# Multi-resolution-diffusion-recommender/SDRM

Measured on AMD Instinct MI355X. Metric: denoising-steps/sec (train+sample) on ML-1M latents, higher is better.
Workload: dtype f32; 1 GPU; ML-1M/MLP shaped synthetic latents (C3/C4); latent=340, width=340, hidden_layers=1, global_batch=8192, n_sample=5429, step_mix=15 train : 78 sample per job cycle, rng=philox4x32-10 on device, sampler_row_chains=2, parallelism=user-sharded dp1, collectives=none

## Files before the change

### include/sdrm_hip_debug.h

```cpp
#ifndef SDRM_HIP_DEBUG_H
#define SDRM_HIP_DEBUG_H

#include "sdrm_hip.h"

#ifdef __cplusplus
extern "C" {
#endif

int sdrm_debug_device_check(const char* gcn_arch, int compute_units);

int sdrm_debug_input_layer_args(int n_items, int hidden, int64_t n_rows, int64_t first, int b, int contiguous, float p_drop,
                                uint32_t* thr, float* scale);

int sdrm_debug_latent_args(int hidden, int latent, int b, int64_t row0, int contiguous);

int sdrm_debug_decoder_nll_args(int latent, int hidden, int n_items, int b, int64_t row0, int64_t n_rows, int contiguous);

int sdrm_debug_vae_adam_args(const uint64_t* addr, const int64_t* n, const float* l2_coef, int n_tensors, int64_t step, int has_partials,
                             int64_t l2_capacity, int64_t* chunks_out);

int sdrm_debug_holdout_args(int n_items, int64_t n_rows, int64_t nnz, double test_prop, int64_t n_u, int64_t* m_out);

int sdrm_debug_vae_eval_args(int n_items, int hidden, int latent, int64_t n_rows, int batch, int k, int metric);

enum { SDRM_TILE_AUTO = -1, SDRM_TILE_COUNT = 5 };

int sdrm_debug_set_tile(sdrm_engine* e, int cfg);
int sdrm_debug_set_nt32_rows(sdrm_engine* e, int max_rows, int max_rows_train);
int sdrm_debug_set_skinny(sdrm_engine* e, int on);
int sdrm_debug_set_rowchain(sdrm_engine* e, int mode);
int sdrm_debug_set_rows48(sdrm_engine* e, int mode);
int sdrm_debug_set_rows48_split(sdrm_engine* e, int mode);
int sdrm_debug_rows48_split_available(const sdrm_engine* e);
int sdrm_debug_set_rows48_share(sdrm_engine* e, int on);
int sdrm_debug_set_sample_persist(sdrm_engine* e, int mode);
int sdrm_debug_split_skew(sdrm_engine* e, unsigned skew);
int sdrm_debug_set_wgrad_strips(sdrm_engine* e, int on);
int sdrm_debug_set_dgrad_rows(sdrm_engine* e, int mode);
int sdrm_debug_rowchain_available(const sdrm_engine* e);
int sdrm_debug_set_fused_reverse(sdrm_engine* e, int mode);
int sdrm_debug_set_chains(sdrm_engine* e, int chains);
int sdrm_debug_chains(const sdrm_engine* e);

enum { SDRM_PLAN_PER_LAYER = 0,
       SDRM_PLAN_SKINNY = 1,
       SDRM_PLAN_ROW96 = 2,
       SDRM_PLAN_ROW48 = 3 };
enum { SDRM_PLAN_DGRAD_TILES = 0,
       SDRM_PLAN_DGRAD_ROWS_PER_LAYER = 1,
       SDRM_PLAN_DGRAD_CHAIN = 2,
       SDRM_PLAN_DGRAD_SKINNY_OWN = 3 };
enum { SDRM_SAMPLE_PATH_SKINNY = 0,
       SDRM_SAMPLE_PATH_PERSIST = 1,
       SDRM_SAMPLE_PATH_PER_LAYER = 2 };
int sdrm_debug_last_plan(const sdrm_engine* e, int* train_path, int* parts, int* dgrad, int* sample_path);

int sdrm_debug_set_gradient_buckets(sdrm_engine* e, int buckets);

int sdrm_debug_philox_draws(sdrm_engine* e, uint64_t seed, uint32_t purpose, uint32_t step, int64_t row0, int rows, int quads,
                            float* normals, uint8_t* lowbits, void* stream);

void* sdrm_debug_comm_handle(const sdrm_engine* e);

int sdrm_debug_plan_wgrad(int rows, int n_out, int k_in, int* slices, int* rows_per_slice);

int sdrm_debug_gemm(int variant, int cfg, const float* A, const float* B, float* C, int M, int N, int K, void* stream);
int sdrm_debug_gemm_time(int variant, int cfg, int M, int N, int K, int reps, float* us_out, void* stream);

int sdrm_debug_svd_args(int64_t m, int64_t n, int64_t nnz, int k, int n_iter);
int sdrm_debug_csr_transpose_args(int64_t m, int64_t n, int64_t capacity);
int sdrm_debug_set_csrt_mark(sdrm_engine* e, int mode);
int sdrm_debug_svd_stage(sdrm_engine* e, const int64_t* indptr, const int32_t* indices, const float* data, int64_t n_rows, int64_t n_cols,
                         int64_t nnz, const float* q, float* y_prod, float* y_orth, void* stream);

int sdrm_debug_neumf_args(int n_users, int n_items, int factor, int64_t listed_users, int64_t listed_items);

int sdrm_debug_neumf_train_args(int n_users, int n_items, int factor, int64_t n, int batch, int64_t step0, float p_drop);

int sdrm_debug_neumf_draw_args(int64_t n, int64_t n_hold, int64_t capacity, int with_present, int n_users);

int sdrm_debug_mlp_train_args(int n_users, int n_items, int64_t n, int batch, int64_t step0, float p_drop, int with_grads, const uint64_t* addr,
                              int n_addr);

int sdrm_debug_mlp_eval_args(int n_users, int n_items, int64_t nnz, int64_t n_rows, int rows_listed, int64_t row0, int64_t n, int batch, int with_out,
                             int with_sse, const uint64_t* addr, int n_addr);

#ifdef __cplusplus
}
// ... 3 lines not shown
```

### sdrm_amd/_lib.py

```python
from __future__ import annotations

import ctypes as C
import os

from . import _build

_LIB = None

c_void_p, c_int, c_int64, c_uint64, c_float = C.c_void_p, C.c_int, C.c_int64, C.c_uint64, C.c_float


class TrainRandoms(C.Structure):
    _fields_ = [("noise", c_void_p), ("t", c_void_p), ("keep", c_void_p)]


class VaeDecoder(C.Structure):
    _fields_ = [("w1", c_void_p), ("b1", c_void_p), ("w2", c_void_p), ("b2", c_void_p), ("latent", c_int), ("hidden", c_int),
                ("n_items", c_int)]


class VaeAdamTensor(C.Structure):
    _fields_ = [("p", c_void_p), ("g", c_void_p), ("m", c_void_p), ("v", c_void_p), ("n", c_int64), ("l2_coef", c_float)]


# ... 135 lines not shown
    "sdrm_debug_philox_draws": (c_int, [c_void_p, c_uint64, C.c_uint32, C.c_uint32, c_int64, c_int, c_int, c_void_p, c_void_p, c_void_p]),
    "sdrm_debug_device_check": (c_int, [C.c_char_p, c_int]),
    "sdrm_debug_input_layer_args": (c_int, [c_int, c_int, c_int64, c_int64, c_int, c_int, c_float, C.POINTER(C.c_uint32), C.POINTER(c_float)]),
    "sdrm_debug_latent_args": (c_int, [c_int, c_int, c_int, c_int64, c_int]),
    "sdrm_debug_decoder_nll_args": (c_int, [c_int, c_int, c_int, c_int, c_int64, c_int64, c_int]),
    "sdrm_debug_vae_adam_args": (c_int, [C.POINTER(c_uint64), C.POINTER(c_int64), C.POINTER(c_float), c_int, c_int64, c_int, c_int64,
                                         C.POINTER(c_int64)]),
    "sdrm_debug_vae_eval_args": (c_int, [c_int, c_int, c_int, c_int64, c_int, c_int, c_int]),
    "sdrm_debug_svd_args": (c_int, [c_int64, c_int64, c_int64, c_int, c_int]),
    "sdrm_debug_csr_transpose_args": (c_int, [c_int64, c_int64, c_int64]),
    "sdrm_debug_set_csrt_mark": (c_int, [c_void_p, c_int]),
    "sdrm_debug_svd_stage": (c_int, [c_void_p, c_void_p, c_void_p, c_void_p, c_int64, c_int64, c_int64, c_void_p, c_void_p, c_void_p, c_void_p]),
    "sdrm_debug_neumf_args": (c_int, [c_int, c_int, c_int, c_int64, c_int64]),
    "sdrm_debug_neumf_train_args": (c_int, [c_int, c_int, c_int, c_int64, c_int, c_int64, c_float]),
    "sdrm_debug_neumf_draw_args": (c_int, [c_int64, c_int64, c_int64, c_int, c_int]),
    "sdrm_debug_mlp_train_args": (c_int, [c_int, c_int, c_int64, c_int, c_int64, c_float, c_int, C.POINTER(c_uint64), c_int]),
    "sdrm_debug_mlp_eval_args": (c_int, [c_int, c_int, c_int64, c_int64, c_int, c_int64, c_int64, c_int, c_int, c_int, C.POINTER(c_uint64), c_int]),
    "sdrm_debug_holdout_args": (c_int, [c_int, c_int64, c_int64, C.c_double, c_int64, C.POINTER(c_int64)]),
    "sdrm_debug_set_tile": (c_int, [c_void_p, c_int]),
    "sdrm_debug_set_nt32_rows": (c_int, [c_void_p, c_int, c_int]),
    "sdrm_debug_set_chains": (c_int, [c_void_p, c_int]),
    "sdrm_debug_chains": (c_int, [c_void_p]),
    "sdrm_debug_last_plan": (c_int, [c_void_p, C.POINTER(c_int), C.POINTER(c_int), C.POINTER(c_int), C.POINTER(c_int)]),
    "sdrm_debug_set_fused_reverse": (c_int, [c_void_p, c_int]),
    "sdrm_debug_set_skinny": (c_int, [c_void_p, c_int]),
    "sdrm_debug_set_rowchain": (c_int, [c_void_p, c_int]),
    "sdrm_debug_set_rows48": (c_int, [c_void_p, c_int]),
    "sdrm_debug_set_rows48_split": (c_int, [c_void_p, c_int]),
    "sdrm_debug_rows48_split_available": (c_int, [c_void_p]),
    "sdrm_debug_split_skew": (c_int, [c_void_p, C.c_uint32]),
    "sdrm_debug_set_sample_persist": (c_int, [c_void_p, c_int]),
    "sdrm_debug_set_rows48_share": (c_int, [c_void_p, c_int]),
    "sdrm_debug_rowchain_available": (c_int, [c_void_p]),
    "sdrm_debug_set_wgrad_strips": (c_int, [c_void_p, c_int]),
    "sdrm_debug_set_dgrad_rows": (c_int, [c_void_p, c_int]),
    "sdrm_debug_comm_handle": (c_void_p, [c_void_p]),
    "sdrm_debug_plan_wgrad": (c_int, [c_int, c_int, c_int, C.POINTER(c_int), C.POINTER(c_int)]),
    "sdrm_debug_gemm_time": (c_int, [c_int, c_int, c_int, c_int, c_int, c_int, C.POINTER(c_float), c_void_p]),
    "sdrm_debug_gemm": (c_int, [c_int, c_int, c_void_p, c_void_p, c_void_p, c_int, c_int, c_int, c_void_p]),
}

RNG_EXPLICIT, RNG_PHILOX = 0, 1
STATUS = {0: "SDRM_OK", -1: "SDRM_ERR_ARG", -2: "SDRM_ERR_SHAPE", -3: "SDRM_ERR_HIP", -4: "SDRM_ERR_STATE",
          -5: "SDRM_ERR_NOMEM", -6: "SDRM_ERR_RCCL", -7: "SDRM_ERR_DEVICE"}


def lib_path() -> str:
    return _build.LIB_PATH


def load(build_if_missing: bool = True):
    global _LIB
    if _LIB is not None:
        return _LIB
    try:
        import torch
    except ImportError:
        pass
    path = lib_path()
    override = os.environ.get("SDRM_LIB")
    if override:
        lib = C.CDLL(os.path.abspath(override))
        missing = [name for name in SIGNATURES if not hasattr(lib, name)]
        if missing:
            raise RuntimeError(f"SDRM_LIB={override}: not this ABI, missing {', '.join(missing[:6])}{' ...' if len(missing) > 6 else ''}")
        for name, (res, args) in SIGNATURES.items():
# ... 25 lines not shown
```

### sdrm_amd/csrc/rowchain.h

```cpp
#pragma once
#include <hip/hip_runtime.h>
#include <stdint.h>

#include "bufres.h"
#include "elementwise.h"
#include "gemm.h"
#include "philox.h"
#include "skinny.h"

namespace sdrm {


__host__ __device__ constexpr int rc_lda(int NP) {
  int p = 4;
  while (((NP + p) % 64) != 8 && ((NP + p) % 64) != 24 && ((NP + p) % 64) != 40 && ((NP + p) % 64) != 56) p += 4;
  return NP + p;
}

struct RowChainArgs {
  const float* x0; const float* noise; const int64_t* t; const uint8_t* keep;
  const float* sqrt_ab; const float* one_minus_ab;
  const float* tembP;
  int B, L, T, H;
  int mode; uint32_t seed_lo, seed_hi, step; int64_t row0; float nd;
// ... 65 lines not shown
    lds0 = (uint32_t)(((tid >> 3) * LDA + 4 * (tid & 7)) * 4);
    g0 = (uint32_t)(((tid >> 3) * sld + 4 * (tid & 7)) * 4);
    sl = 0u; sg = 0u; jj = 0;
    gwrap = (uint32_t)(RC_USERS * sld * 4 - (CT - 1) * 128);
  }
  template <int CT, int LDA>
  __device__ __forceinline__ void next() {
    const bool wrap = jj == CT - 1;
    jj = wrap ? 0 : jj + 1;
    sl += wrap ? (uint32_t)(RC_USERS * LDA * 4 - (CT - 1) * 128) : 128u;
    sg += wrap ? gwrap : 128u;
  }
};

template <int CT>
__device__ __forceinline__ void rc_acc_begin(f32x4 (&acc)[3][CT]) {
#pragma unroll
  for (int rt = 0; rt < 3; ++rt)
#pragma unroll
    for (int ct = 0; ct < CT; ++ct) asm volatile("" : "+a"(acc[rt][ct]));
  asm volatile("s_nop 7");
}
template <int CT>
__device__ __forceinline__ void rc_acc_settle(f32x4 (&acc)[3][CT]) {
  asm volatile("s_nop 15\n\ts_nop 15" : "+a"(acc[0][0]));
#pragma unroll
  for (int rt = 0; rt < 3; ++rt)
#pragma unroll
    for (int ct = 0; ct < CT; ++ct)
      if (rt + ct > 0) asm volatile("" : "+a"(acc[rt][ct]));
}

enum { RC_PLAIN = 0, RC_NEXT_LIGHT = 1, RC_LIGHT = 2 };
template <int CT, int LDA, int NS, bool STREAM, bool NT, int MODE = RC_PLAIN, int RTS = RC_USERS>
__device__ __forceinline__ void rc_kstep(f32x4 (&acc)[3][CT], const f32x4 (&ac)[3], const f32x4 (&bc)[CT], f32x4 (&an)[3],
                                         f32x4 (&bn)[CT], brsrc wres, uint32_t wnext, uint32_t lane16, uint32_t anext,
                                         const float* __restrict__ Act, brsrc sres, RcStream& sw) {
  constexpr int NE = MODE == RC_LIGHT ? 1 : 4;
  constexpr int NSLOT = 3 * NE * CT;
  constexpr int P_A = MODE == RC_LIGHT ? 0 : CT, P_S = MODE == RC_LIGHT ? 0 : CT + 3, NPIECE = P_S + (STREAM ? 2 * NS : 0);
  constexpr int STRIDE = NPIECE == 0 ? NSLOT : (NSLOT / NPIECE >= RC_PIECE_STRIDE ? RC_PIECE_STRIDE : (NSLOT / NPIECE >= 1 ? NSLOT / NPIECE : 1));
  static_assert(NPIECE <= NSLOT && NS <= 2, "not enough MFMA slots for the pipeline pieces");
  f32x4 sv0 = {0.f, 0.f, 0.f, 0.f}, sv1 = sv0;
  uint32_t so0 = 0, so1 = 0;
#pragma unroll
  for (int e = 0; e < NE; ++e)
#pragma unroll
  for (int ct = 0; ct < CT; ++ct)
#pragma unroll
  for (int rt = 0; rt < 3; ++rt) {
    const int s = (e * CT + ct) * 3 + rt;
    asm volatile("v_mfma_f32_16x16x4_f32 %0, %1, %2, %0" : "+a"(acc[rt][ct]) : "v"(bc[ct][e]), "v"(ac[rt][e]));
    if (s % STRIDE == 0 && s / STRIDE < NPIECE) {
      const int p = s / STRIDE;
      if (p < P_A) {
        if (!(RC_DIAG & 2)) {
          uint32_t so = wnext + (p / 4) * 4096;
          asm volatile("" : "+s"(so));
          bn[p] = bload4(wres, lane16 + (p % 4) * 1024, so);
        }
      } else if (p < P_S) {
        if (!(RC_DIAG & 4)) {
          uint32_t ao = anext;
          asm volatile("" : "+v"(ao));
          if (MODE == RC_NEXT_LIGHT) an[p - P_A][0] = *reinterpret_cast<const float*>(reinterpret_cast<const char*>(Act) + ao + (p - P_A) * RTS * LDA * 4);
          else an[p - P_A] = *reinterpret_cast<const f32x4*>(reinterpret_cast<const char*>(Act) + ao + (p - P_A) * RTS * LDA * 4);
        }
      } else {
        constexpr int NSD = NS > 0 ? NS : 1;
        const int k = p - P_S, ph = k / NSD, q = k % NSD;
        if (!(RC_DIAG & 1)) {
          f32x4& v = q == 0 ? sv0 : sv1;
          uint32_t& so = q == 0 ? so0 : so1;
          if (ph == 0) {
            uint32_t lo = sw.lds0 + sw.sl;
            asm volatile("" : "+v"(lo));
            v = *reinterpret_cast<const f32x4*>(reinterpret_cast<const char*>(Act) + lo);
            so = sw.sg;
            sw.template next<CT, LDA>();
          } else {
            asm volatile("" : "+s"(so));
            bstore4<NT>(sres, sw.g0, so, v);
          }
        }
      }
    }
    __builtin_amdgcn_sched_barrier(0);
  }
}

__device__ __forceinline__ void block_sum4(double (&v)[4], double* sh ) {
#pragma unroll
  for (int j = 0; j < 4; ++j)
#pragma unroll
    for (int off = 32; off > 0; off >>= 1) v[j] += __shfl_down(v[j], off, 64);
  const int lane = threadIdx.x & 63, wave = threadIdx.x >> 6;
  __syncthreads();
  if (lane == 0) {
#pragma unroll
    for (int j = 0; j < 4; ++j) sh[4 * wave + j] = v[j];
  }
  __syncthreads();
#pragma unroll
  for (int j = 0; j < 4; ++j) v[j] = (sh[j] + sh[4 + j]) + (sh[8 + j] + sh[12 + j]);
}

template <int CT, bool LIGHT = false>
__global__ __launch_bounds__(NTHREADS, 1) void k_row_fwd(const RowChainArgs a) {
  typedef RowChainCfg<CT> C;
  constexpr int NP = C::NP, NCT = C::NCT, KS = C::KS, QP = C::QP, LDA = C::LDA, RT = 3;
  static_assert(KS % 2 == 0, "K-steps are taken in pairs");
  __shared__ __attribute__((aligned(16))) float Act[RC_ROWS * LDA];
  __shared__ int trow[RC_USERS];
  __shared__ double red[16];
  const int tid = threadIdx.x, lane = tid & 63;
  const int wave = __builtin_amdgcn_readfirstlane(tid >> 6);
  const int wr = wave >> 1, wc = wave & 1;
  const int li = lane & 15, lq = lane >> 4;
  const int g = blockIdx.x, u0 = RC_USERS * g;
  const size_t grow0 = (size_t)RC_ROWS * g;
#ifdef RC_STAMPS
  unsigned long long st_[16] = {0};
#endif
  RC_STAMP(0);

  if (tid < RC_USERS) {
    const int usr = u0 + tid;
    int t0 = 0;
    if (usr < a.B) {
      t0 = train_timestep(a.mode, a.t, a.row0, usr, a.step, a.seed_lo, a.seed_hi, a.T);
      a.tdev[usr] = t0;
    }
    trow[tid] = t0;
  }
  constexpr int NQ = QP / 8;
  const int su = tid >> 3, sq = tid & 7;
  const int susr = u0 + su;
  float4 xs[NQ];
#pragma unroll
  for (int j = 0; j < NQ; ++j) {
    const int c = 4 * (sq + 8 * j);
    xs[j] = (susr < a.B && c < a.L) ? load4_unpadded(a.x0, susr, c, a.L) : make_float4(0.f, 0.f, 0.f, 0.f);
  }
  __syncthreads();
  {
    const int TPc = a.K0 - a.LPs;
    const int TQ8 = TPc >> 5;
    const bool uin = susr < a.B;
    const float* trow_p = a.tembP + (size_t)(uin ? trow[su] : 0) * TPc + 4 * sq;
    const brsrc ures = make_brsrc(a.U + grow0 * a.K0, (uint32_t)(RC_ROWS * a.K0 * 4));
    const uint32_t uvo = (uint32_t)((su * a.K0 + a.LPs + 4 * sq) * 4);
    for (int jq = 0; jq < TQ8; ++jq) {
      const float4 te = uin ? *reinterpret_cast<const float4*>(trow_p + 32 * jq) : make_float4(0.f, 0.f, 0.f, 0.f);
      const f32x4 oh = {te.x, te.y, te.z, te.w};
#pragma unroll
      for (int pass = 0; pass < 3; ++pass) bstore4<true>(ures, uvo, (uint32_t)((pass * RC_USERS * a.K0 + 32 * jq) * 4), oh);
    }
  }
  {
    const int tt = trow[su];
    const float sa = a.sqrt_ab[tt], om = a.one_minus_ab[tt];
    U4 rw[NQ];
    if (a.mode != 0) {
#pragma unroll
      for (int j = 0; j < NQ; ++j)
        rw[j] = train_quad_draw(a.row0, susr, sq + 8 * j, a.step, a.seed_lo, a.seed_hi);
    }
#pragma unroll
    for (int j = 0; j < NQ; ++j) {
      const int c = 4 * (sq + 8 * j);
      float vP[4] = {0.f, 0.f, 0.f, 0.f}, vS[4] = {0.f, 0.f, 0.f, 0.f}, vQ[4] = {0.f, 0.f, 0.f, 0.f};
      if (susr < a.B && c < a.L) {
        const float x_[4] = {xs[j].x, xs[j].y, xs[j].z, xs[j].w};
        float e[4] = {0.f, 0.f, 0.f, 0.f};
        uint32_t bits[4] = {0u, 0u, 0u, 0u};
        if (a.mode != 0) {
          train_quad_decode(rw[j], a.nd, e, bits);
        }
#pragma unroll
        for (int k = 0; k < 4; ++k) {
          if (c + k < a.L) {
            const size_t idx = (size_t)susr * a.L + c + k;
            const float x = x_[k];
            bool k1, k2, k3;
            float ee;
            if (a.mode == 0) {
              ee = a.noise[idx];
              const size_t BL = (size_t)a.B * a.L;
              k1 = a.keep[idx] != 0; k2 = a.keep[BL + idx] != 0; k3 = a.keep[2 * BL + idx] != 0;
            } else {
              ee = e[k];
              k1 = bits[k] & 1u; k2 = (bits[k] >> 1) & 1u; k3 = (bits[k] >> 2) & 1u;
            }
            stage_element(x, ee, sa, om, k1, k2, k3, vP[k], vS[k], vQ[k]);
          }
        }
      }
      if (c == (a.ones_col & ~3)) {
#pragma unroll
        for (int k = 0; k < 4; ++k)
          if (k == (a.ones_col & 3)) vP[k] = vS[k] = vQ[k] = 1.f;
      }
      *reinterpret_cast<float4*>(Act + su * LDA + c) = make_float4(vP[0], vP[1], vP[2], vP[3]);
      *reinterpret_cast<float4*>(Act + (RC_USERS + su) * LDA + c) = make_float4(vS[0], vS[1], vS[2], vS[3]);
      *reinterpret_cast<float4*>(Act + (2 * RC_USERS + su) * LDA + c) = make_float4(vQ[0], vQ[1], vQ[2], vQ[3]);
    }
  }
  __syncthreads();
  RC_STAMP(1);

  const float* abase = Act + (16 * wr + li) * LDA + 4 * lq;
  const uint32_t aoff = (uint32_t)(((16 * wr + li) * LDA + 4 * lq) * 4);
  const uint32_t aoffl = (uint32_t)(((16 * wr + li) * LDA + lq) * 4);
  const uint32_t lane16 = 16u * (uint32_t)lane;
  const int myrow = 16 * wr + li;
  const int mycol = 16 * CT * wc + 4 * lq;
  float* __restrict__ otile = Act + myrow * LDA + mycol;
  f32x4 acc[RT][CT];
  f32x4 b0[CT], b1[CT];
  f32x4 a0[RT], a1[RT];
  f32x4 xq[CT];

  const int nlayers = a.H + 2;
  for (int layer = 0; layer < nlayers; ++layer) {
    const bool last = layer == nlayers - 1;
    const brsrc Wf = make_brsrc((layer == 0 ? a.W0f : (last ? a.Wof : a.Whf)) + (size_t)(CT * wc) * 256, (uint32_t)((KS * NCT - CT * wc) * 1024));
    const bool stream = layer == 0 || a.act != nullptr;
    float* sdst = layer == 0 ? a.U + grow0 * a.K0 : a.act + (size_t)(layer - 1) * a.pre_stride + grow0 * a.ldp;
    const int sld = layer == 0 ? a.K0 : a.ldp;
    const brsrc sres = make_brsrc(stream ? sdst : a.U, stream ? (uint32_t)(RC_ROWS * sld * 4) : 0u);

    {
      const float* bsrc = layer == 0 ? a.B0tab + (size_t)trow[myrow] * a.ldtab : (last ? a.bo : a.bh);
#pragma unroll
      for (int ct = 0; ct < CT; ++ct) {
        const float4 bv = *reinterpret_cast<const float4*>(bsrc + mycol + 16 * ct);
#pragma unroll
        for (int rt = 0; rt < RT; ++rt) acc[rt][ct] = f32x4{bv.x, bv.y, bv.z, bv.w};
      }
    }
    if (last) {
      const int usr = u0 + myrow;
#pragma unroll
      for (int ct = 0; ct < CT; ++ct) {
        const int col = mycol + 16 * ct;
        const float4 x = (usr < a.B && col < a.L) ? load4_unpadded(a.x0, usr, col, a.L) : make_float4(0.f, 0.f, 0.f, 0.f);
        xq[ct] = f32x4{x.x, x.y, x.z, x.w};
      }
    }
#pragma unroll
    for (int ct = 0; ct < CT; ++ct) b0[ct] = bload4(Wf, lane16 + ct * 1024u, 0u);
#pragma unroll
    for (int rt = 0; rt < RT; ++rt) a0[rt] = *reinterpret_cast<const f32x4*>(abase + rt * RC_USERS * LDA);
    RcStream sw;
    sw.template init<CT, LDA>(tid, sld);
    auto kloop = [&](auto stream_tag, auto nt_tag) {
      constexpr bool STREAM = decltype(stream_tag)::value, NT = decltype(nt_tag)::value;
      constexpr uint32_t WS = NCT * 1024;
      for (uint32_t ks = 0; ks < (uint32_t)KS - 2; ks += 2) {
        rc_kstep<CT, LDA, 2, STREAM, NT>(acc, a0, b0, a1, b1, Wf, (ks + 1) * WS, lane16, aoff + 64u * (ks + 1), Act, sres, sw);
        rc_kstep<CT, LDA, 1, STREAM, NT>(acc, a1, b1, a0, b0, Wf, (ks + 2) * WS, lane16, aoff + 64u * (ks + 2), Act, sres, sw);
      }
      if constexpr (LIGHT) {
        rc_kstep<CT, LDA, 2, STREAM, NT, RC_NEXT_LIGHT>(acc, a0, b0, a1, b1, Wf, (KS - 1) * WS, lane16, aoffl + 64u * (KS - 1), Act, sres, sw);
        rc_kstep<CT, LDA, 1, STREAM, NT, RC_LIGHT>(acc, a1, b1, a0, b0, Wf, 0u, lane16, aoff, Act, sres, sw);
      } else {
        rc_kstep<CT, LDA, 2, STREAM, NT>(acc, a0, b0, a1, b1, Wf, (KS - 1) * WS, lane16, aoff + 64u * (KS - 1), Act, sres, sw);
        rc_kstep<CT, LDA, 1, STREAM, NT>(acc, a1, b1, a0, b0, Wf, (KS - 2) * WS, lane16, aoff + 64u * (KS - 2), Act, sres, sw);
      }
    };
    rc_acc_begin<CT>(acc);
    if (stream) kloop(std::true_type{}, std::true_type{});
    else kloop(std::false_type{}, std::false_type{});
    rc_acc_settle<CT>(acc);
    if (layer < 3) RC_STAMP(2 + 3 * layer);
    if (last) break;

    __syncthreads();
    if (layer < 3) RC_STAMP(3 + 3 * layer);
    {
      const float slope = layer == 0 ? *a.slope0 : *a.slopeh;
      gchar* pw = uniform_gptr(a.pre + (size_t)layer * a.pre_stride + grow0 * a.ldp);
      const uint32_t pbase = (uint32_t)((myrow * a.ldp + mycol) * 4);
      const uint32_t prt = (uint32_t)(RC_USERS * a.ldp * 4);
      if (!(a.skip_pre && slope >= SLOPE_FROM_ACT_MIN)) {
#pragma unroll
        for (int rt = 0; rt < RT; ++rt)
#pragma unroll
          for (int ct = 0; ct < CT; ++ct) {
            const f32x4 v = acc[rt][ct];
            if (!(RC_DIAG & 8)) gstore4(pw + ct * 64, pbase + rt * prt, make_float4(v[0], v[1], v[2], v[3]));
          }
      }
#pragma unroll
      for (int rt = 0; rt < RT; ++rt)
#pragma unroll
        for (int ct = 0; ct < CT; ++ct) {
          const f32x4 v = acc[rt][ct];
          *reinterpret_cast<float4*>(otile + rt * RC_USERS * LDA + 16 * ct) =
              make_float4(prelu_any(v[0], slope), prelu_any(v[1], slope), prelu_any(v[2], slope), prelu_any(v[3], slope));
        }
// ... 8 lines not shown
  double sD = 0, sC = 0, sR = 0, sR2 = 0;
#pragma unroll
  for (int ct = 0; ct < CT; ++ct) {
    const int col = mycol + 16 * ct;
    float fD = 0.f, fC = 0.f, fR = 0.f, fR2 = 0.f;
    float P[4], S[4], Q[4];
#pragma unroll
    for (int i = 0; i < 4; ++i) { P[i] = tanh_fast(acc[0][ct][i]); S[i] = tanh_fast(acc[1][ct][i]); Q[i] = tanh_fast(acc[2][ct][i]); }
    gstore4(yw + ct * 64, ybase, make_float4(P[0], P[1], P[2], P[3]));
    gstore4(yw + ct * 64, ybase + yrt, make_float4(S[0], S[1], S[2], S[3]));
    gstore4(yw + ct * 64, ybase + 2 * yrt, make_float4(Q[0], Q[1], Q[2], Q[3]));
#pragma unroll
    for (int i = 0; i < 4; ++i) {
      if (uok && col + i < a.L) loss_terms<true>(P[i], S[i], Q[i], xq[ct][i], fD, fC, fR, fR2);
    }
    sD += fD; sC += fC; sR += fR; sR2 += fR2;
  }
  RC_STAMP(9);
  double tot[4] = {sD, sC, sR, sR2};
  block_sum4(tot, red);
  if (tid == 0) {
    double* o = a.loss_part + 4 * (size_t)g;
    o[0] = tot[0]; o[1] = tot[1]; o[2] = tot[2]; o[3] = tot[3];
  }
#ifdef RC_STAMPS
  RC_STAMP(10);
  if (tid == 0 && a.stamps) {
    st_[12] = __builtin_amdgcn_s_memrealtime();
    for (int i = 0; i < 16; ++i) a.stamps[16 * (size_t)g + i] = st_[i];
  }
#endif
}

}
```

### sdrm_amd/csrc/sdrm_hip.hip

```cpp
#include <hip/hip_runtime.h>

#include <algorithm>
#include <cmath>
#include <cstdio>
#include <cstdlib>
#include <cstring>
#include <mutex>
#include <set>
#include <string>
#include <type_traits>
#include <utility>
#include <vector>

#include "../../include/sdrm_hip.h"
#include "../../include/sdrm_hip_debug.h"
#include "compact.h"
#include "csr_transpose.h"
#include "decode.h"
#include "decoder_train.h"
#include "elementwise.h"
#include "encode.h"
#include "eval_half.h"
#include "exchange.h"
#include "feed.h"
// ... 953 lines not shown
                       uint64_t seed, uint64_t step, float nd, hipStream_t st) {
  const int n = e->T + 1, G = p.groups;
  RowChainArgs a{};
  a.x0 = x0;
  if (mode == SDRM_RNG_EXPLICIT) { a.noise = rnd->noise; a.t = rnd->t; a.keep = rnd->keep; }
  a.sqrt_ab = e->sched + 3 * n; a.one_minus_ab = e->sched + 4 * n; a.tembP = e->tembP;
  a.B = p.B; a.L = e->L; a.T = e->T; a.H = e->H;
  a.mode = mode; a.seed_lo = (uint32_t)seed; a.seed_hi = (uint32_t)(seed >> 32); a.step = (uint32_t)step; a.row0 = row0; a.nd = nd;
  a.W0f = e->W0f; a.Whf = e->Whf; a.Wof = e->Wof; a.bh = e->bhc; a.bo = e->boc; a.B0tab = e->B0tab; a.ldtab = e->WP;
  a.slope0 = slope_ptr(e, 0); a.slopeh = e->H > 0 ? slope_ptr(e, 1) : slope_ptr(e, 0);
  a.U = e->U; a.K0 = e->K0; a.LPs = e->LP; a.tdev = e->tdev; a.ones_col = e->ones_col;
  a.light = rc_light_klast(e->W, e->WP) >= 0 ? 1 : 0;
  a.pre = e->pre; a.pre_stride = (size_t)e->MPmax * e->WP; a.ldp = e->WP; a.Y = e->Y; a.ldy = e->LP;
  a.act = e->act;
  a.loss_part = e->loss_part;
  a.sweep = (e->tune.rows48_share & 4) ? 1 : 0;
  a.skip_pre = p.skip_pre() ? 1 : 0;
  const double flops = 2.0 * 3 * a.B * ((double)e->W * e->L + (double)e->H * e->W * e->W + (double)e->L * e->W);
  if (p.path == StepPlan::ROW48) {
    if (p.parts > 1) {
      if (int rc = split_sync(e, false, G, p.parts, e->H + 1, st, &a.xcnt, &a.xbase)) return rc;
      a.xabort = e->xabort_dev; a.ngroups = G;
    }
    const int grid = rows48_grid(G, p.parts);
    return with_rows48_form(e, p.parts, (e->tune.rows48_share & 1) != 0, [&](auto ct, auto light, auto np, auto share) {
      return hip_rc(e, "k_rows48_fwd", profiled(e, PC_ROW_FWD, flops, st, [&] {
        SDRM_LAUNCH(e, (k_rows48_fwd<VAL(ct), VAL(light), VAL(np), VAL(share)>), dim3((unsigned)grid), dim3(NTHREADS), 0, st, a);
        return hipGetLastError();
      }));
    });
  }
  return with_row_form(e, [&](auto ct, auto light) {
    return hip_rc(e, "k_row_fwd", profiled(e, PC_ROW_FWD, flops, st, [&] {
      SDRM_LAUNCH(e, (k_row_fwd<VAL(ct), VAL(light)>), dim3((unsigned)G), dim3(NTHREADS), 0, st, a);
      return hipGetLastError();
    }));
  });
}

SkStepArgs sk_step_args(sdrm_engine* e, int B) {
  SkStepArgs a{};
  const int n = e->T + 1;
  a.W0c = e->W0c; a.K0 = e->K0; a.Whc = e->Whc; a.Woc = e->Woc; a.bh = e->bhc; a.bo = e->boc;
  a.WhcT = e->WhcT; a.WocT = e->WocT; a.B0tab = e->B0tab;
  a.WeP = e->WeP; a.W0eP = e->W0eP; a.be = e->p + e->off_be; a.b0 = e->b0c; a.TPe = e->TPe; a.intab = e->WeP ? 1 : 0;
  a.slope0 = slope_ptr(e, 0); a.slopeh = e->H > 0 ? slope_ptr(e, 1) : slope_ptr(e, 0);
  a.sqrt_ab = e->sched + 3 * n; a.one_minus_ab = e->sched + 4 * n; a.tembP = e->tembP;
  a.B = B; a.L = e->L; a.W = e->W; a.T = e->T; a.H = e->H; a.G = (B + SK_USERS - 1) / SK_USERS;
  a.LPs = e->LP; a.WPs = e->WP; a.TPs = e->TP;
  a.U = e->U; a.tdev = e->tdev; a.pre = e->pre; a.pre_stride = (size_t)e->MPmax * e->WP; a.Y = e->Y;
  a.loss_part = e->loss_part; a.NP = a.G;
  a.slab0 = e->slab0; a.slabH = e->slabH; a.slabO = e->slabO; a.db0s = e->db0s; a.dbHs = e->dbHs; a.dbOs = e->dbOs;
  a.alpha_part = e->alpha_part; a.alpha_part_stride = e->alpha_part_stride;
  return a;
}

template <int NL, int NW>
int launch_sk_step_nlnw(sdrm_engine* e, const SkStepArgs& ka, int which, int grid, hipStream_t st) {
  typedef SkCfg<NL, NW> C;
  const size_t lds = (which == 0 ? sk_fwd_lds_floats<NL, NW>(ka.intab ? ka.TPe : 0) : sk_bwd_lds_floats<NL, NW>(ka.TPs)) * sizeof(float);
  if (lds > 48 * 1024) HIP_TRY(e, allow_full_lds(which == 0 ? (const void*)k_skinny_fwd<NL, NW> : (const void*)k_skinny_bwd<NL, NW>));
  if (which == 0) SDRM_LAUNCH(e, (k_skinny_fwd<NL, NW>), dim3((unsigned)grid), dim3(C::NTHR), lds, st, ka);
  else SDRM_LAUNCH(e, (k_skinny_bwd<NL, NW>), dim3((unsigned)grid), dim3(C::NTHR), lds, st, ka);
  HIP_TRY(e, hipGetLastError());
  return SDRM_OK;
}

// ... 514 lines not shown
  if (B < 1 || B > e->max_rows) return fail(e, SDRM_ERR_SHAPE, "sdrm_train_forward: B outside [1, max_rows]");
  if (mode == SDRM_RNG_EXPLICIT && (!rnd || !rnd->noise || !rnd->t || !rnd->keep))
    return fail(e, SDRM_ERR_ARG, "sdrm_train_forward: EXPLICIT mode needs noise, t and keep");
  if (mode != SDRM_RNG_EXPLICIT && mode != SDRM_RNG_PHILOX) return fail(e, SDRM_ERR_ARG, "bad rng mode");
  hipStream_t st = (hipStream_t)stream;
  e->bwd_begun = false;
  if (int cr = chains_train_forward(e, st)) return cr;
  e->fwd_done = false;
  e->fwd_params_live = true;
  if (int xs = split_status(e)) return xs;
  e->plan = plan_step(e, B);
  StepPlan& p = e->plan;
  if (p.path == StepPlan::SKINNY) {
    int rc = e->WeP ? SDRM_OK : ensure_tables(e, st);
    if (rc) return rc;
    SkStepArgs ka = sk_step_args(e, B);
    ka.x0 = x0;
    if (mode == SDRM_RNG_EXPLICIT) { ka.noise = rnd->noise; ka.t = rnd->t; ka.keep = rnd->keep; }
    ka.mode = mode; ka.seed_lo = (uint32_t)seed; ka.seed_hi = (uint32_t)(seed >> 32); ka.step = (uint32_t)step;
    ka.row0 = row0; ka.nd = nd;
    bool done4 = false;
    if (e->tune.skinny == 1) {
      ka.NP = 4 * ka.G;
      rc = launch_sk_fwd4(e, ka, st, &done4);
      if (rc) return rc;
    }
    if (!done4) {
      ka.NP = ka.G;
      rc = launch_sk_step(e, ka, 0, ka.G, st);
      if (rc) return rc;
    }
    p.loss_parts = ka.NP;
  } else if (p.path == StepPlan::ROW96 || p.path == StepPlan::ROW48) {
    int rc = emb_tables(e, st, x0, (size_t)B * e->L);
    if (rc) return rc;
    rc = launch_row_forward(e, p, x0, row0, mode, rnd, seed, step, nd, st);
    if (rc) return rc;
    chains_train_row_owned(e);
  } else {
    const int MP = p.MP, n = e->T + 1;
    const int cfg = choose_cfg(e->tune, MP, e->tune.nt32_max_rows_train);
    PrepTrainArgs pa{};
    pa.x0 = x0;
    if (mode == SDRM_RNG_EXPLICIT) { pa.noise = rnd->noise; pa.t = rnd->t; pa.keep = rnd->keep; }
    pa.sqrt_ab = e->sched + 3 * n; pa.one_minus_ab = e->sched + 4 * n; pa.tembP = e->tembP;
    pa.U = e->U; pa.tdev = e->tdev;
    pa.B = B; pa.L = e->L; pa.LP = e->LP; pa.K0 = e->K0; pa.T = e->T; pa.MP = MP;
    pa.mode = mode; pa.seed_lo = (uint32_t)seed; pa.seed_hi = (uint32_t)(seed >> 32); pa.step = (uint32_t)step;
    pa.row0 = row0; pa.nd = nd;
    {
      pa.emb = emb_args(e);
      e->tables_fresh = true;
      pa.emb_row0 = B + (MP - 3 * B);
      pa.emb_chunks = (e->WP + 63) / 64;
      pa.emb_blocks = (e->T + 1) * pa.emb_chunks;
      const int main_blocks = (int)(((int64_t)pa.emb_row0 * (e->K0 / 4) + 255) / 256);
      SDRM_LAUNCH(e, k_prep_train, dim3(pa.emb_blocks + main_blocks), dim3(256), 2 * e->T * sizeof(float), st, pa);
      HIP_TRY(e, hipGetLastError());
    }
    {
      GemmArgs a{};
      a.C = pre_buf(e, 0); a.ldc = e->WP; a.bias = e->B0tab; a.ldtab = e->WP; a.trow = e->tdev; a.trow_B = B;
      HIP_TRY(e, (gemm_forward<XF_NONE, EPI_BIAS_ROWTAB>(a, e->U, e->K0, e->W0c, e->K0, MP, e->WP, e->LP, st,
                                                         Prof{e, PC_FWD_L0, 2.0 * 3 * B * (double)e->W * e->L}, cfg)));
    }
    int rc = hidden_forward(e, MP, 3 * B, st, cfg);
    if (rc) return rc;
// ... 411 lines not shown
  const int buckets = e->tune.ar_buckets == 2 ? 2 : 1;
  if (buckets == 1) {
    rc = sdrm_train_backward(e, e->sums, nullptr, loss, stream);
    if (rc) return rc;
    NCCL_TRY(e, api, api->AllReduce(e->g, e->g, (size_t)e->P, ncclFloat, ncclSum, x.comm, st));
    return sdrm_adam_step(e, nullptr, lr, stream);
  }
  rc = sdrm_train_backward_begin(e, e->sums, nullptr, loss, stream);
  if (rc) return rc;
  const int64_t n0 = e->off_a0, n1 = e->P - e->off_a0;
  HIP_TRY(e, hipEventRecord(x.ev_bucket, st));
  HIP_TRY(e, hipStreamWaitEvent(x.aux, x.ev_bucket, 0));
  NCCL_TRY(e, api, api->AllReduce(e->g, e->g, (size_t)n0, ncclFloat, ncclSum, x.comm, x.aux));
  rc = sdrm_train_backward_finish(e, nullptr, stream);
  if (rc) return rc;
  HIP_TRY(e, hipEventRecord(x.ev_bucket, st));
  HIP_TRY(e, hipStreamWaitEvent(x.aux, x.ev_bucket, 0));
  NCCL_TRY(e, api, api->AllReduce(e->g + n0, e->g + n0, (size_t)n1, ncclFloat, ncclSum, x.comm, x.aux));
  HIP_TRY(e, hipEventRecord(x.ev_done, x.aux));
  HIP_TRY(e, hipStreamWaitEvent(st, x.ev_done, 0));
  return sdrm_adam_step(e, nullptr, lr, stream);
}

int sdrm_get_train_outputs(const sdrm_engine* e, float* psq, void* stream) {
  if (!e || !psq) return SDRM_ERR_ARG;
  sdrm_engine* me = const_cast<sdrm_engine*>(e);
  if (!e->fwd_done) return fail(me, SDRM_ERR_STATE, "sdrm_get_train_outputs: no forward yet");
  SDRM_LAUNCH(e, k_unpad_psq, dim3(256), dim3(256), 0, (hipStream_t)stream, (const float*)e->Y, e->plan.B, e->L,
                     e->LP, e->plan.order, psq);
  HIP_TRY(me, hipGetLastError());
  return SDRM_OK;
}

static int forward_rows(sdrm_engine* e, const float* x, const int64_t* t, int t_uniform, int n, int mode,
                        const uint8_t* keep, uint64_t seed, uint64_t step, int64_t row0, float* out, int ldout,
                        int cols_valid, hipStream_t st) {
  if (int jr = chains_join(e, st)) return jr;
  const int MP = round_up(n, BM);
  const int cfg = choose_cfg(e->tune, MP, e->tune.nt32_max_rows);
  PrepFwdArgs pa{};
  pa.x = x; pa.t = t; pa.t_uniform = t_uniform; pa.keep = keep; pa.U = e->U;
  pa.n = n; pa.L = e->L; pa.LP = e->LP; pa.K0 = e->K0; pa.T = e->T; pa.MP = MP;
  pa.mode = mode; pa.seed_lo = (uint32_t)seed; pa.seed_hi = (uint32_t)(seed >> 32); pa.step = (uint32_t)step;
  pa.row0 = row0;
  pa.bpr = (e->K0 / 2 + 255) / 256;
  dim3 grid((unsigned)((size_t)pa.bpr * MP));
  SDRM_LAUNCH(e, k_prep_forward, grid, dim3(256), 0, st, pa);
  HIP_TRY(e, hipGetLastError());
  int rc = ensure_tables(e, st);
  if (rc) return rc;
  {
    GemmArgs a{};
    a.C = pre_buf(e, 0); a.ldc = e->WP; a.bias = e->b0c;
    HIP_TRY(e, (gemm_forward<XF_NONE, EPI_BIAS>(a, e->U, e->K0, e->W0c, e->K0, MP, e->WP, e->K0, st,
                                                Prof{e, PC_FWD_L0, 2.0 * n * (double)e->W * (e->L + e->T)}, cfg)));
  }
  rc = hidden_forward(e, MP, n, st, cfg);
  if (rc) return rc;
  GemmArgs a{};
  a.C = out; a.ldc = ldout; a.bias = e->boc; a.slopeA = slope_ptr(e, e->H);
  a.rows_valid = n; a.cols_valid = cols_valid;
  HIP_TRY(e, (gemm_forward<XF_PRELU, EPI_BIAS_TANH_G>(a, pre_buf(e, e->H), e->WP, e->Woc, e->WP, MP, e->LP, e->WP, st,
                                                    Prof{e, PC_FWD_OUT, 2.0 * n * (double)e->L * e->W}, cfg)));
  return SDRM_OK;
}

// ... 2398 lines not shown
```

### sdrm_amd/engine.py

```python
from __future__ import annotations

import collections
import ctypes as C
import math
import os
import weakref

import numpy as np
import torch

from . import _lib, synth


class SdrmError(RuntimeError):
    pass


def _ptr(t):
    return None if t is None else C.c_void_p(t.data_ptr())


def _stream():
    return C.c_void_p(torch.cuda.current_stream().cuda_stream)

# ... 273 lines not shown
        return buf.raw

    def comm_init_rank(self, nranks: int, rank: int, unique_id: bytes):
        if len(unique_id) != 128:
            raise SdrmError("comm_init_rank: the unique id is 128 bytes")
        self._check(self.lib.sdrm_comm_init_rank(self._h, int(nranks), int(rank), C.c_char_p(unique_id)), "sdrm_comm_init_rank")
        return self

    def comm_info(self):
        n, r = C.c_int(), C.c_int()
        self._check(self.lib.sdrm_comm_info(self._h, C.byref(n), C.byref(r)), "sdrm_comm_info")
        return int(n.value), int(r.value)

    def train_step_sharded(self, x0, lr, row0=0, noise=None, t=None, keep=None, seed=0, step=0, nd=1.0):
        x0 = self._dev(x0, torch.float32)
        B = x0.shape[0]
        if x0.dim() != 2 or x0.shape[1] != self.L:
            raise SdrmError(f"train_step_sharded: x0 must be [B,{self.L}]")
        self._x0 = x0
        if noise is not None:
            rnd = self._randoms(noise, t, keep, B)
            rc = self.lib.sdrm_train_step_sharded(self._h, _ptr(x0), B, int(row0), float(lr), _lib.RNG_EXPLICIT, C.byref(rnd),
                                                  0, 0, float(nd), _ptr(self._loss), _stream())
        else:
            rc = self.lib.sdrm_train_step_sharded(self._h, _ptr(x0), B, int(row0), float(lr), _lib.RNG_PHILOX, None, int(seed),
                                                  int(step), float(nd), _ptr(self._loss), _stream())
        self._check(rc, "sdrm_train_step_sharded")
        return self._loss

    def train_outputs(self, B):
        out = torch.empty(3, B, self.L, dtype=torch.float32, device=self.device)
        self._check(self.lib.sdrm_get_train_outputs(self._h, _ptr(out), _stream()), "sdrm_get_train_outputs")
        return out

    def preacts(self, layer, B):
        out = torch.empty(3, B, self.W, dtype=torch.float32, device=self.device)
        self._check(self.lib.sdrm_get_preacts(self._h, int(layer), _ptr(out), _stream()), "sdrm_get_preacts")
        return out

    def launch_count(self):
        return int(self.lib.sdrm_launch_count(self._h))

    def profile_begin(self, capacity=4096, only=None):
        cls = -1
        if only is not None:
            names = [self.lib.sdrm_profile_name(c).decode() for c in range(self.lib.sdrm_profile_classes())]
            cls = names.index(only)
        self._check(self.lib.sdrm_profile_only(self._h, cls), "sdrm_profile_only")
        self._check(self.lib.sdrm_profile_begin(self._h, int(capacity)), "sdrm_profile_begin")

    def profile_end(self):
        self._check(self.lib.sdrm_profile_end(self._h, _stream()), "sdrm_profile_end")
        out = {}
        for c in range(self.lib.sdrm_profile_classes()):
            ms, n, fl = C.c_double(), C.c_int64(), C.c_double()
            self._check(self.lib.sdrm_profile_get(self._h, c, C.byref(ms), C.byref(n), C.byref(fl)), "sdrm_profile_get")
            if n.value:
                out[self.lib.sdrm_profile_name(c).decode()] = (ms.value, int(n.value), fl.value)
        return out

    def forward(self, x, t, keep=None, seed=0, step=0, row0=0):
        x = self._dev(x, torch.float32)
        t = self._dev(t, torch.int64)
        n = x.shape[0]
        out = torch.empty(n, self.L, dtype=torch.float32, device=self.device)
        if keep is not None:
# ... 1029 lines not shown
```

Before: 9247 denoising-steps/s.

## Restructure row-chain forward prologue and use running A-fragment offsets

The row-chain forward kernel is split into Philox and explicit-RNG variants so the mode branch is resolved at compile time. Its prologue is reordered: the x0 loads go through buffer resources, timesteps are computed per thread without a barrier, time-embedding rows are prefetched ahead, and staging uses masked vector ops. The K-loop now advances A-fragment offsets with running counters plus immediate offsets to save address arithmetic. The emb_tables warm-up is also skipped on the ROW96 path. A debug accessor for the staged activations is added for validation. The risks are higher register pressure and small numeric differences from the changed FMA contraction.

New measurement: 9356 denoising-steps/s, median of 6. 1.2% higher.

```diff
diff --git a/include/sdrm_hip_debug.h b/include/sdrm_hip_debug.h
--- a/include/sdrm_hip_debug.h
+++ b/include/sdrm_hip_debug.h
@@ -54,6 +54,7 @@
        SDRM_SAMPLE_PATH_PERSIST = 1,
        SDRM_SAMPLE_PATH_PER_LAYER = 2 };
 int sdrm_debug_last_plan(const sdrm_engine* e, int* train_path, int* parts, int* dgrad, int* sample_path);
+int sdrm_debug_get_staged(const sdrm_engine* e, float* staged, int* t, void* stream);
 
 int sdrm_debug_set_gradient_buckets(sdrm_engine* e, int buckets);
 
diff --git a/sdrm_amd/_lib.py b/sdrm_amd/_lib.py
--- a/sdrm_amd/_lib.py
+++ b/sdrm_amd/_lib.py
@@ -191,6 +191,7 @@
     "sdrm_debug_set_sample_persist": (c_int, [c_void_p, c_int]),
     "sdrm_debug_set_rows48_share": (c_int, [c_void_p, c_int]),
     "sdrm_debug_rowchain_available": (c_int, [c_void_p]),
+    "sdrm_debug_get_staged": (c_int, [c_void_p, c_void_p, c_void_p, c_void_p]),
     "sdrm_debug_set_wgrad_strips": (c_int, [c_void_p, c_int]),
     "sdrm_debug_set_dgrad_rows": (c_int, [c_void_p, c_int]),
     "sdrm_debug_comm_handle": (c_void_p, [c_void_p]),
diff --git a/sdrm_amd/csrc/rowchain.h b/sdrm_amd/csrc/rowchain.h
--- a/sdrm_amd/csrc/rowchain.h
+++ b/sdrm_amd/csrc/rowchain.h
@@ -121,10 +121,10 @@
 }
 
 enum { RC_PLAIN = 0, RC_NEXT_LIGHT = 1, RC_LIGHT = 2 };
-template <int CT, int LDA, int NS, bool STREAM, bool NT, int MODE = RC_PLAIN, int RTS = RC_USERS>
+template <int CT, int LDA, int NS, bool STREAM, bool NT, int MODE = RC_PLAIN, int RTS = RC_USERS, int AIMM = -1>
 __device__ __forceinline__ void rc_kstep(f32x4 (&acc)[3][CT], const f32x4 (&ac)[3], const f32x4 (&bc)[CT], f32x4 (&an)[3],
                                          f32x4 (&bn)[CT], brsrc wres, uint32_t wnext, uint32_t lane16, uint32_t anext,
-                                         const float* __restrict__ Act, brsrc sres, RcStream& sw) {
+                                         const float* __restrict__ Act, brsrc sres, RcStream& sw, uint32_t* arun = nullptr) {
   constexpr int NE = MODE == RC_LIGHT ? 1 : 4;
   constexpr int NSLOT = 3 * NE * CT;
   constexpr int P_A = MODE == RC_LIGHT ? 0 : CT, P_S = MODE == RC_LIGHT ? 0 : CT + 3, NPIECE = P_S + (STREAM ? 2 * NS : 0);
@@ -150,10 +150,17 @@
         }
       } else if (p < P_S) {
         if (!(RC_DIAG & 4)) {
-          uint32_t ao = anext;
-          asm volatile("" : "+v"(ao));
-          if (MODE == RC_NEXT_LIGHT) an[p - P_A][0] = *reinterpret_cast<const float*>(reinterpret_cast<const char*>(Act) + ao + (p - P_A) * RTS * LDA * 4);
-          else an[p - P_A] = *reinterpret_cast<const f32x4*>(reinterpret_cast<const char*>(Act) + ao + (p - P_A) * RTS * LDA * 4);
+          if constexpr (AIMM >= 0) {
+            static_assert(MODE == RC_PLAIN, "running offsets are those of the plain fragment layout");
+            uint32_t& ar = arun[p - P_A == 2 ? 1 : 0];
+            asm volatile("" : "+v"(ar));
+            an[p - P_A] = *reinterpret_cast<const f32x4*>(reinterpret_cast<const char*>(Act) + ar + AIMM + (p - P_A == 1 ? RTS * LDA * 4 : 0));
+          } else {
+            uint32_t ao = anext;
+            asm volatile("" : "+v"(ao));
+            if (MODE == RC_NEXT_LIGHT) an[p - P_A][0] = *reinterpret_cast<const float*>(reinterpret_cast<const char*>(Act) + ao + (p - P_A) * RTS * LDA * 4);
+            else an[p - P_A] = *reinterpret_cast<const f32x4*>(reinterpret_cast<const char*>(Act) + ao + (p - P_A) * RTS * LDA * 4);
+          }
         }
       } else {
         constexpr int NSD = NS > 0 ? NS : 1;
@@ -194,8 +201,29 @@
   for (int j = 0; j < 4; ++j) v[j] = (sh[j] + sh[4 + j]) + (sh[8 + j] + sh[12 + j]);
 }
 
-template <int CT, bool LIGHT = false>
-__global__ __launch_bounds__(NTHREADS, 1) void k_row_fwd(const RowChainArgs a) {
+typedef uint32_t u32x4 __attribute__((ext_vector_type(4)));
+
+__device__ __forceinline__ uint32_t rc_keep_mask(uint32_t w, int p) { return (uint32_t)((int32_t)(w << (31 - p)) >> 31); }
+
+template <bool FMA0>
+__device__ __forceinline__ void rc_stage_quad(f32x4 X, f32x4 E, float sa, float om, const uint32_t (&kw)[4], f32x4& P, f32x4& S, f32x4& Q) {
+#pragma clang fp contract(off)
+  const f32x4 oe = om * E;
+  f32x4 p = sa * X + oe;
+  if (FMA0) p[0] = __builtin_fmaf(sa, X[0], oe[0]);
+  p = 2.f * p;
+  const f32x4 s = 2.f * X;
+  const f32x4 q = 2.f * __builtin_elementwise_fma(E, f32x4{MU, MU, MU, MU}, X);
+  u32x4 mP, mS, mQ;
+#pragma unroll
+  for (int k = 0; k < 4; ++k) { mP[k] = rc_keep_mask(kw[k], 0); mS[k] = rc_keep_mask(kw[k], 1); mQ[k] = rc_keep_mask(kw[k], 2); }
+  P = __builtin_bit_cast(f32x4, __builtin_bit_cast(u32x4, p) & mP);
+  S = __builtin_bit_cast(f32x4, __builtin_bit_cast(u32x4, s) & mS);
+  Q = __builtin_bit_cast(f32x4, __builtin_bit_cast(u32x4, q) & mQ);
+}
+
+template <int CT, bool LIGHT, bool PHILOX>
+__device__ __forceinline__ void row_fwd_body(const RowChainArgs& a) {
   typedef RowChainCfg<CT> C;
   constexpr int NP = C::NP, NCT = C::NCT, KS = C::KS, QP = C::QP, LDA = C::LDA, RT = 3;
   static_assert(KS % 2 == 0, "K-steps are taken in pairs");
@@ -213,87 +241,110 @@
 #endif
   RC_STAMP(0);
 
-  if (tid < RC_USERS) {
-    const int usr = u0 + tid;
-    int t0 = 0;
-    if (usr < a.B) {
-      t0 = train_timestep(a.mode, a.t, a.row0, usr, a.step, a.seed_lo, a.seed_hi, a.T);
-      a.tdev[usr] = t0;
-    }
-    trow[tid] = t0;
-  }
   constexpr int NQ = QP / 8;
   const int su = tid >> 3, sq = tid & 7;
   const int susr = u0 + su;
-  float4 xs[NQ];
+  const bool live = susr < a.B;
+  f32x4 xs[NQ];
+  {
+    const brsrc xres = make_brsrc(a.x0 + (size_t)u0 * a.L, (uint32_t)(min(max(a.B - u0, 0), RC_USERS) * a.L * 4));
+    constexpr uint32_t BEYOND = 0x7ffffff0u;
+    const uint32_t xrow = (uint32_t)(su * a.L * 4);
+    if ((a.L & 3) == 0) {
+#pragma unroll
+      for (int j = 0; j < NQ; ++j) {
+        const int c = 4 * (sq + 8 * j);
+        xs[j] = bload4(xres, c < a.L ? xrow + 4u * c : BEYOND, 0u);
+      }
+    } else {
+#pragma unroll
+      for (int j = 0; j < NQ; ++j)
+#pragma unroll
+        for (int k = 0; k < 4; ++k) {
+          const int c = 4 * (sq + 8 * j) + k;
+          xs[j][k] = bload1(xres, c < a.L ? xrow + 4u * c : BEYOND, 0u);
+        }
+    }
+  }
+  int tt = 0;
+  if constexpr (PHILOX) {
+    const int td = train_timestep(1, nullptr, a.row0, susr, a.step, a.seed_lo, a.seed_hi, a.T);
+    tt = live ? td : 0;
+  } else {
+    if (live) tt = train_timestep(0, a.t, a.row0, susr, a.step, a.seed_lo, a.seed_hi, a.T);
+  }
+  if (sq == 0) {
+    trow[su] = tt;
+    if (live) a.tdev[susr] = tt;
+  }
+  const float sa = a.sqrt_ab[tt], om = a.one_minus_ab[tt];
+  const int TPc = a.K0 - a.LPs;
+  const int TQ8 = TPc >> 5;
+  constexpr int TE_AHEAD = 4;
+  constexpr uint32_t TE_BEYOND = 0x7ffffff0u;
+  const brsrc tres = make_brsrc(a.tembP, (uint32_t)((a.T + 1) * TPc * 4));
+  const uint32_t tvo = live ? (uint32_t)((tt * TPc + 4 * sq) * 4) : TE_BEYOND;
+  f32x4 te[TE_AHEAD];
+#pragma unroll
+  for (int jq = 0; jq < TE_AHEAD; ++jq) te[jq] = bload4(tres, jq < TQ8 ? tvo + 128u * jq : TE_BEYOND, 0u);
+  U4 rw[NQ];
+  if constexpr (PHILOX) {
+#pragma unroll
+    for (int j = 0; j < NQ; ++j) rw[j] = train_quad_draw(a.row0, susr, sq + 8 * j, a.step, a.seed_lo, a.seed_hi);
+#pragma unroll
+    for (int j = 0; j < NQ; ++j) asm volatile("" : : "v"(rw[j].x));
+  }
+  {
+    const brsrc ures = make_brsrc(a.U + grow0 * a.K0, (uint32_t)(RC_ROWS * a.K0 * 4));
+    const uint32_t uvo = (uint32_t)((su * a.K0 + a.LPs + 4 * sq) * 4);
+#pragma unroll
+    for (int jq = 0; jq < TE_AHEAD; ++jq)
+#pragma unroll
+      for (int pass = 0; pass < 3; ++pass)
+        bstore4<true>(ures, jq < TQ8 ? uvo + 128u * jq : TE_BEYOND, (uint32_t)(pass * RC_USERS * a.K0 * 4), te[jq]);
+    for (int jq = TE_AHEAD; jq < TQ8; ++jq) {
+      const f32x4 oh = bload4(tres, tvo, 128u * jq);
+#pragma unroll
+      for (int pass = 0; pass < 3; ++pass) bstore4<true>(ures, uvo, (uint32_t)((pass * RC_USERS * a.K0 + 32 * jq) * 4), oh);
+    }
+  }
 #pragma unroll
   for (int j = 0; j < NQ; ++j) {
     const int c = 4 * (sq + 8 * j);
-    xs[j] = (susr < a.B && c < a.L) ? load4_unpadded(a.x0, susr, c, a.L) : make_float4(0.f, 0.f, 0.f, 0.f);
-  }
-  __syncthreads();
-  {
-    const int TPc = a.K0 - a.LPs;
-    const int TQ8 = TPc >> 5;
-    const bool uin = susr < a.B;
-    const float* trow_p = a.tembP + (size_t)(uin ? trow[su] : 0) * TPc + 4 * sq;
-    const brsrc ures = make_brsrc(a.U + grow0 * a.K0, (uint32_t)(RC_ROWS * a.K0 * 4));
-    const uint32_t uvo = (uint32_t)((su * a.K0 + a.LPs + 4 * sq) * 4);
-    for (int jq = 0; jq < TQ8; ++jq) {
-      const float4 te = uin ? *reinterpret_cast<const float4*>(trow_p + 32 * jq) : make_float4(0.f, 0.f, 0.f, 0.f);
-      const f32x4 oh = {te.x, te.y, te.z, te.w};
-#pragma unroll
-      for (int pass = 0; pass < 3; ++pass) bstore4<true>(ures, uvo, (uint32_t)((pass * RC_USERS * a.K0 + 32 * jq) * 4), oh);
-    }
-  }
-  {
-    const int tt = trow[su];
-    const float sa = a.sqrt_ab[tt], om = a.one_minus_ab[tt];
-    U4 rw[NQ];
-    if (a.mode != 0) {
-#pragma unroll
-      for (int j = 0; j < NQ; ++j)
-        rw[j] = train_quad_draw(a.row0, susr, sq + 8 * j, a.step, a.seed_lo, a.seed_hi);
-    }
-#pragma unroll
-    for (int j = 0; j < NQ; ++j) {
-      const int c = 4 * (sq + 8 * j);
-      float vP[4] = {0.f, 0.f, 0.f, 0.f}, vS[4] = {0.f, 0.f, 0.f, 0.f}, vQ[4] = {0.f, 0.f, 0.f, 0.f};
-      if (susr < a.B && c < a.L) {
-        const float x_[4] = {xs[j].x, xs[j].y, xs[j].z, xs[j].w};
-        float e[4] = {0.f, 0.f, 0.f, 0.f};
-        uint32_t bits[4] = {0u, 0u, 0u, 0u};
-        if (a.mode != 0) {
-          train_quad_decode(rw[j], a.nd, e, bits);
-        }
-#pragma unroll
-        for (int k = 0; k < 4; ++k) {
-          if (c + k < a.L) {
-            const size_t idx = (size_t)susr * a.L + c + k;
-            const float x = x_[k];
-            bool k1, k2, k3;
-            float ee;
-            if (a.mode == 0) {
-              ee = a.noise[idx];
-              const size_t BL = (size_t)a.B * a.L;
-              k1 = a.keep[idx] != 0; k2 = a.keep[BL + idx] != 0; k3 = a.keep[2 * BL + idx] != 0;
-            } else {
-              ee = e[k];
-              k1 = bits[k] & 1u; k2 = (bits[k] >> 1) & 1u; k3 = (bits[k] >> 2) & 1u;
-            }
-            stage_element(x, ee, sa, om, k1, k2, k3, vP[k], vS[k], vQ[k]);
-          }
-        }
-      }
-      if (c == (a.ones_col & ~3)) {
-#pragma unroll
-        for (int k = 0; k < 4; ++k)
-          if (k == (a.ones_col & 3)) vP[k] = vS[k] = vQ[k] = 1.f;
-      }
-      *reinterpret_cast<float4*>(Act + su * LDA + c) = make_float4(vP[0], vP[1], vP[2], vP[3]);
-      *reinterpret_cast<float4*>(Act + (RC_USERS + su) * LDA + c) = make_float4(vS[0], vS[1], vS[2], vS[3]);
-      *reinterpret_cast<float4*>(Act + (2 * RC_USERS + su) * LDA + c) = make_float4(vQ[0], vQ[1], vQ[2], vQ[3]);
-    }
+    const int nvalid = live ? min(max(a.L - c, 0), 4) : 0;
+    const f32x4 X = xs[j];
+    f32x4 E;
+    uint32_t kw[4];
+    if constexpr (PHILOX) {
+      float e[4];
+      train_quad_decode(rw[j], a.nd, e, kw);
+      E = f32x4{e[0], e[1], e[2], e[3]};
+    } else {
+      const size_t idx = (size_t)susr * a.L + c, BL = (size_t)a.B * a.L;
+#pragma unroll
+      for (int k = 0; k < 4; ++k) {
+        E[k] = 0.f; kw[k] = 0u;
+        if (k < nvalid) {
+          E[k] = a.noise[idx + k];
+          kw[k] = (a.keep[idx + k] != 0 ? 1u : 0u) | (a.keep[BL + idx + k] != 0 ? 2u : 0u) | (a.keep[2 * BL + idx + k] != 0 ? 4u : 0u);
+        }
+      }
+    }
+    if (PHILOX && nvalid < 4) {
+#pragma unroll
+      for (int k = 0; k < 4; ++k)
+        if (k >= nvalid) kw[k] = 0u;
+    }
+    f32x4 vP, vS, vQ;
+    rc_stage_quad<CT == 11>(X, E, sa, om, kw, vP, vS, vQ);
+    if (c == (a.ones_col & ~3)) {
+#pragma unroll
+      for (int k = 0; k < 4; ++k)
+        if (k == (a.ones_col & 3)) vP[k] = vS[k] = vQ[k] = 1.f;
+    }
+    *reinterpret_cast<f32x4*>(Act + su * LDA + c) = vP;
+    *reinterpret_cast<f32x4*>(Act + (RC_USERS + su) * LDA + c) = vS;
+    *reinterpret_cast<f32x4*>(Act + (2 * RC_USERS + su) * LDA + c) = vQ;
   }
   __syncthreads();
   RC_STAMP(1);
@@ -346,16 +397,18 @@
     auto kloop = [&](auto stream_tag, auto nt_tag) {
       constexpr bool STREAM = decltype(stream_tag)::value, NT = decltype(nt_tag)::value;
       constexpr uint32_t WS = NCT * 1024;
+      uint32_t arun[2] = {aoff, aoff + (uint32_t)(2 * RC_USERS * LDA * 4)};
       for (uint32_t ks = 0; ks < (uint32_t)KS - 2; ks += 2) {
-        rc_kstep<CT, LDA, 2, STREAM, NT>(acc, a0, b0, a1, b1, Wf, (ks + 1) * WS, lane16, aoff + 64u * (ks + 1), Act, sres, sw);
-        rc_kstep<CT, LDA, 1, STREAM, NT>(acc, a1, b1, a0, b0, Wf, (ks + 2) * WS, lane16, aoff + 64u * (ks + 2), Act, sres, sw);
+        rc_kstep<CT, LDA, 2, STREAM, NT, RC_PLAIN, RC_USERS, 64>(acc, a0, b0, a1, b1, Wf, (ks + 1) * WS, lane16, 0u, Act, sres, sw, arun);
+        rc_kstep<CT, LDA, 1, STREAM, NT, RC_PLAIN, RC_USERS, 128>(acc, a1, b1, a0, b0, Wf, (ks + 2) * WS, lane16, 0u, Act, sres, sw, arun);
+        arun[0] += 128u; arun[1] += 128u;
       }
       if constexpr (LIGHT) {
         rc_kstep<CT, LDA, 2, STREAM, NT, RC_NEXT_LIGHT>(acc, a0, b0, a1, b1, Wf, (KS - 1) * WS, lane16, aoffl + 64u * (KS - 1), Act, sres, sw);
         rc_kstep<CT, LDA, 1, STREAM, NT, RC_LIGHT>(acc, a1, b1, a0, b0, Wf, 0u, lane16, aoff, Act, sres, sw);
       } else {
-        rc_kstep<CT, LDA, 2, STREAM, NT>(acc, a0, b0, a1, b1, Wf, (KS - 1) * WS, lane16, aoff + 64u * (KS - 1), Act, sres, sw);
-        rc_kstep<CT, LDA, 1, STREAM, NT>(acc, a1, b1, a0, b0, Wf, (KS - 2) * WS, lane16, aoff + 64u * (KS - 2), Act, sres, sw);
+        rc_kstep<CT, LDA, 2, STREAM, NT, RC_PLAIN, RC_USERS, 64>(acc, a0, b0, a1, b1, Wf, (KS - 1) * WS, lane16, 0u, Act, sres, sw, arun);
+        rc_kstep<CT, LDA, 1, STREAM, NT, RC_PLAIN, RC_USERS, 0>(acc, a1, b1, a0, b0, Wf, (KS - 2) * WS, lane16, 0u, Act, sres, sw, arun);
       }
     };
     rc_acc_begin<CT>(acc);
@@ -430,4 +483,9 @@
 #endif
 }
 
-}
+template <int CT, bool LIGHT = false>
+__global__ __launch_bounds__(NTHREADS, 1) void k_row_fwd(const RowChainArgs a) { row_fwd_body<CT, LIGHT, true>(a); }
+template <int CT, bool LIGHT = false>
+__global__ __launch_bounds__(NTHREADS, 1) void k_row_fwd_explicit(const RowChainArgs a) { row_fwd_body<CT, LIGHT, false>(a); }
+
+}
diff --git a/sdrm_amd/csrc/sdrm_hip.hip b/sdrm_amd/csrc/sdrm_hip.hip
--- a/sdrm_amd/csrc/sdrm_hip.hip
+++ b/sdrm_amd/csrc/sdrm_hip.hip
@@ -1009,7 +1009,8 @@
   }
   return with_row_form(e, [&](auto ct, auto light) {
     return hip_rc(e, "k_row_fwd", profiled(e, PC_ROW_FWD, flops, st, [&] {
-      SDRM_LAUNCH(e, (k_row_fwd<VAL(ct), VAL(light)>), dim3((unsigned)G), dim3(NTHREADS), 0, st, a);
+      if (mode == SDRM_RNG_EXPLICIT) SDRM_LAUNCH(e, (k_row_fwd_explicit<VAL(ct), VAL(light)>), dim3((unsigned)G), dim3(NTHREADS), 0, st, a);
+      else SDRM_LAUNCH(e, (k_row_fwd<VAL(ct), VAL(light)>), dim3((unsigned)G), dim3(NTHREADS), 0, st, a);
       return hipGetLastError();
     }));
   });
@@ -1590,7 +1591,8 @@
     }
     p.loss_parts = ka.NP;
   } else if (p.path == StepPlan::ROW96 || p.path == StepPlan::ROW48) {
-    int rc = emb_tables(e, st, x0, (size_t)B * e->L);
+    const bool warm = p.path == StepPlan::ROW48;
+    int rc = emb_tables(e, st, warm ? x0 : nullptr, warm ? (size_t)B * e->L : 0);
     if (rc) return rc;
     rc = launch_row_forward(e, p, x0, row0, mode, rnd, seed, step, nd, st);
     if (rc) return rc;
@@ -2068,6 +2070,18 @@
   return SDRM_OK;
 }
 
+int sdrm_debug_get_staged(const sdrm_engine* e, float* staged, int* t, void* stream) {
+  if (!e) return SDRM_ERR_ARG;
+  sdrm_engine* me = const_cast<sdrm_engine*>(e);
+  if (!e->fwd_done) return fail(me, SDRM_ERR_STATE, "sdrm_debug_get_staged: no forward yet");
+  if (staged) {
+    SDRM_LAUNCH(e, k_unpad_psq, dim3(256), dim3(256), 0, (hipStream_t)stream, (const float*)e->U, e->plan.B, e->L, e->K0, e->plan.order, staged);
+    HIP_TRY(me, hipGetLastError());
+  }
+  if (t) HIP_TRY(me, hipMemcpyAsync(t, e->tdev, (size_t)e->plan.B * sizeof(int), hipMemcpyDeviceToDevice, (hipStream_t)stream));
+  return SDRM_OK;
+}
+
 static int forward_rows(sdrm_engine* e, const float* x, const int64_t* t, int t_uniform, int n, int mode,
                         const uint8_t* keep, uint64_t seed, uint64_t step, int64_t row0, float* out, int ldout,
                         int cols_valid, hipStream_t st) {
diff --git a/sdrm_amd/engine.py b/sdrm_amd/engine.py
--- a/sdrm_amd/engine.py
+++ b/sdrm_amd/engine.py
@@ -329,6 +329,12 @@
         out = torch.empty(3, B, self.L, dtype=torch.float32, device=self.device)
         self._check(self.lib.sdrm_get_train_outputs(self._h, _ptr(out), _stream()), "sdrm_get_train_outputs")
         return out
+
+    def staged(self, B):
+        out = torch.empty(3, B, self.L, dtype=torch.float32, device=self.device)
+        t = torch.empty(B, dtype=torch.int32, device=self.device)
+        self._check(self.lib.sdrm_debug_get_staged(self._h, _ptr(out), _ptr(t), _stream()), "sdrm_debug_get_staged")
+        return out, t
 
     def preacts(self, layer, B):
         out = torch.empty(3, B, self.W, dtype=torch.float32, device=self.device)
```
